# CobayaSampler/cobaya

Measured on AMD Instinct MI355X. Metric: log-posterior evals/sec (whole node), 30-dim gaussian_mixture, higher is better.
Workload: dtype f64

## Files before the change

### cobaya_amd/csrc/_exp/inc_experiment.h

```cpp
#pragma once
#include <hip/hip_runtime.h>

#define MCMC_EXP_FAMILY_STEP 0
#define MCMC_EXP_FAMILY_DRAG 1
#define MCMC_EXP_FAMILY_MIX 2
#ifndef EXP_STEP_WAVES
#define EXP_STEP_WAVES 0
#endif
#ifndef EXP_DRAG_WAVES
#define EXP_DRAG_WAVES 0
#endif
#ifndef EXP_MIX_WAVES
#define EXP_MIX_WAVES 0
#endif
#define MCMC_EXP_WAVES(family, tuned)                                                     \
    ((MCMC_EXP_FAMILY_##family == 0 && EXP_STEP_WAVES) ? EXP_STEP_WAVES                    \
     : (MCMC_EXP_FAMILY_##family == 1 && EXP_DRAG_WAVES) ? EXP_DRAG_WAVES                  \
     : (MCMC_EXP_FAMILY_##family == 2 && EXP_MIX_WAVES) ? EXP_MIX_WAVES : (tuned))
#ifdef EXP_PIPE
#define MCMC_EXP_PIPE(tuned) (EXP_PIPE)
#else
#define MCMC_EXP_PIPE(tuned) (tuned)
#endif
#ifdef EXP_ROTATE_SHIFT
#define MCMC_EXP_ROTATE_SHIFT(tuned) (EXP_ROTATE_SHIFT)
#else
#define MCMC_EXP_ROTATE_SHIFT(tuned) (tuned)
#endif
#ifdef EXP_KEEP
#define MCMC_EXP_KEEP(tuned) (EXP_KEEP != 0)
#else
#define MCMC_EXP_KEEP(tuned) (tuned)
#endif
#ifdef EXP_BOUNDS_REGS
#define MCMC_EXP_BOUNDS_LDS(tuned) (false)
#endif
#ifdef EXP_FLOAT_BOUNDS
#define MCMC_EXP_FLOAT_BOUNDS(tuned) (true)
#endif
#ifdef EXP_NO_ROTATE
#define MCMC_EXP_ROTATE(on) (false)
#else
#define MCMC_EXP_ROTATE(on) (on)
#endif

#ifdef EXP_BLOCK_TIMES
__device__ unsigned long long g_block_times[2 * 4096];
__device__ unsigned int g_wave_place[2 * 4 * 4096];
extern "C" __attribute__((visibility("default"))) int mcmc_hip_debug_block_times(unsigned long long* out)
{
    return (int)hipMemcpyFromSymbol(out, HIP_SYMBOL(g_block_times), sizeof(g_block_times));
}
extern "C" __attribute__((visibility("default"))) int mcmc_hip_debug_wave_place(unsigned int* out)
{
    return (int)hipMemcpyFromSymbol(out, HIP_SYMBOL(g_wave_place), sizeof(g_wave_place));
}
#define MCMC_EXP_BLOCK_BEGIN()                                                                \
    do {                                                                                      \
        if (threadIdx.x == 0 && blockIdx.x < 4096) g_block_times[2 * blockIdx.x] = wall_clock64(); \
        if ((threadIdx.x & 63) == 0 && blockIdx.x < 4096) {                                   \
            g_wave_place[2 * (4 * blockIdx.x + (threadIdx.x >> 6))] =                         \
                __builtin_amdgcn_s_getreg((4) | (0 << 6) | (31 << 11));                       \
            g_wave_place[2 * (4 * blockIdx.x + (threadIdx.x >> 6)) + 1] =                     \
                __builtin_amdgcn_s_getreg((20) | (0 << 6) | (31 << 11));                      \
        }                                                                                     \
    } while (0)
#define MCMC_EXP_BLOCK_END()                                                                  \
    do {                                                                                      \
        if (threadIdx.x == 0 && blockIdx.x < 4096)                                            \
            g_block_times[2 * blockIdx.x + 1] = wall_clock64();                               \
    } while (0)
#else
#define MCMC_EXP_BLOCK_BEGIN() ((void)0)
#define MCMC_EXP_BLOCK_END() ((void)0)
#endif
#ifdef EXP_FLOAT_LDS
#define MCMC_EXP_FLOAT_LDS(tuned) (EXP_FLOAT_LDS != 0)
#endif
#ifdef EXP_FLOAT_LDS_KEEP
#define MCMC_EXP_FLOAT_LDS_KEEP(tuned) (EXP_FLOAT_LDS_KEEP != 0)
#endif
#ifdef EXP_FLOAT_VEC
#define MCMC_EXP_FLOAT_VEC(tuned) (EXP_FLOAT_VEC != 0)
#endif
#ifdef EXP_DUO_DEPK
#define MCMC_DUO_DEPK(tuned) (EXP_DUO_DEPK)
#endif
#ifdef EXP_DUO_KEEPV
#define MCMC_DUO_KEEPV(tuned) (EXP_DUO_KEEPV != 0)
#endif
```

### cobaya_amd/csrc/incremental_duo.hip

```cpp
#include <string>

#include "incremental_common.h"

#ifndef MCMC_DUO_DEPK
#define MCMC_DUO_DEPK(tuned) (tuned)
#endif
#ifndef MCMC_DUO_KEEPV
#define MCMC_DUO_KEEPV(tuned) (tuned)
#endif

namespace mcmc {
namespace {

__device__ __forceinline__ double pair_swap(double v) { return quad_perm<0xB1>(v); }
__device__ __forceinline__ double duo_sum(double p_even, double p_odd)
{
    const double s = p_even + p_odd;
    return s + pair_swap(s);
}
__device__ __forceinline__ unsigned pair_max_u32(unsigned v)
{
    const unsigned o = (unsigned)__builtin_amdgcn_mov_dpp((int)v, 0xB1, 0xf, 0xf, true);
    return v > o ? v : o;
}
__device__ __forceinline__ unsigned long long pair_all_mask(unsigned long long m)
{
    m &= m >> 1;
    m &= 0x5555555555555555ull;
    return m * 3ull;
}

constexpr int kDuoRow = 33;
constexpr int kDuoStagedPairs = 4 * 8 * kDuoRow;
struct DuoVariates {
    unsigned base, off;
    __device__ __forceinline__ void init(const pair_t* sRE, int wave, int lane)
    {
        base = lds_offset(sRE + (wave * 8 * kDuoRow + (lane >> 1)));
        off = base;
    }
    __device__ __forceinline__ void put(pair_t* sRE, int wave, int lane, int h, int q, const PairRng& p)
    {
        pair_t* const mine = sRE + ((wave * 8 + 4 * h + 2 * q) * kDuoRow + (lane >> 1));
        mine[0] = pair_t{p.r[0], p.Ea[0]};
        mine[kDuoRow] = pair_t{p.r[1], p.Ea[1]};
    }
    __device__ __forceinline__ void seek(unsigned long long S) { off = base + (unsigned)(S & 7ull) * (16u * kDuoRow); }
    __device__ __forceinline__ void fetch(double& r, double& Ea) const
    {
        const pair_t re = *(lds_pairs)(unsigned long long)off;
        r = re.x;
        Ea = re.y;
    }
    __device__ __forceinline__ void next() { off += 16u * kDuoRow; }
};

__host__ __device__ constexpr int duo_chunk_mix(int dq, int km)
{
    const int avail = 80 * 1024 - 16896 - 2560 - 2048 - (duo_x_in_lds(km, dq) ? dq * 4096 : 0);
    int c = ((avail / 16) / ((1 + km) * 4 * dq)) & ~3;
    return c < 4 ? 4 : (c > 64 ? 64 : c);
}
__host__ __device__ constexpr bool duo_keep_v(int dq, int km)
{
    return 2 * dq * (km + (duo_x_in_lds(km, dq) ? 0 : 1)) + 2 * dq <= 64;
}

template <int DQ, int KM, bool UNIT_T, bool BOX0>
__global__ void __launch_bounds__(256, 2) step_duo_mix_kernel(const IncStepArgs a)
{
    extern __shared__ __attribute__((aligned(16))) double smem[];
    constexpr int dpad = 4 * DQ;
    constexpr int NE = 2 * DQ;
    constexpr int COL = (1 + KM) * dpad;
    constexpr int C = duo_chunk_mix(DQ, KM);
    constexpr int CHUNK = C * COL;
    constexpr int DEPK = MCMC_DUO_DEPK(DQ / 2);
    constexpr bool XLDS = duo_x_in_lds(KM, DQ);
    constexpr bool KEEPV = MCMC_DUO_KEEPV(duo_keep_v(DQ, KM));
    const StepArgs& s = a.s;
    const int tid = threadIdx.x, h = tid & 1, wave = tid >> 6, lane = tid & 63;
    const int W = s.W, d = a.d;
    const int w = blockIdx.x * 128 + (tid >> 1);
    const int g = __builtin_amdgcn_readfirstlane(w / s.group_size);
    const int ncols = s.n_steps;
    const double* __restrict__ gVU = a.VU + (size_t)g * ncols * COL;
    auto stage = [&](int k) {
        const int first = k * C;
        if (first >= ncols) return;
        const int cols = ncols - first < C ? ncols - first : C;
        const int bytes = cols * COL * 8;
        const char* src = (const char*)(gVU + (size_t)first * COL);
        char* dst = (char*)(smem + (k & 1) * CHUNK);
        for (int kb = wave; kb * 1024 < bytes; kb += 4) {
            if (kb * 1024 + lane * 16 < bytes)
                __builtin_amdgcn_global_load_lds(
                    (const __attribute__((address_space(1))) void*)(src + kb * 1024 + lane * 16),
                    (__attribute__((address_space(3))) void*)(dst + kb * 1024), 16, 0, 0);
        }
    };
    stage(0);
    __shared__ double2 sLH[BOX0 ? 1 : 4 * DQ];
    __shared__ double2 sNA[BOX0 ? 1 : 4 * DQ];
    __shared__ double sNM[BOX0 ? 1 : 4 * DQ];
    if (!BOX0)
        for (int i = tid; i < dpad; i += 256) {
            sLH[i] = make_double2(a.prior[i], a.prior[dpad + i]);
            sNA[i] = make_double2(a.prior[2 * dpad + i], a.prior[3 * dpad + i]);
            sNM[i] = a.prior[4 * dpad + i];
        }
    double x[XLDS ? 1 : NE], y[KM][NE];
    typedef pair_t __attribute__((address_space(3))) * lds_pairs_rw;
    __shared__ pair_t sX[XLDS ? DQ * 256 : 1];
    const unsigned xoff0 = lds_offset(sX + tid);
#pragma unroll
    for (int kk = 0; kk < DQ; ++kk) {
        double xe[2];
#pragma unroll
        for (int j = 0; j < 2; ++j) {
            const int e = 2 * kk + j, i = 4 * kk + 2 * h + j;
            const bool in = i < d;
            xe[j] = in ? s.x[(size_t)i * W + w] : (BOX0 ? 0.5 * a.box_hi : 0.0);
            if (!XLDS) x[XLDS ? 0 : e] = xe[j];
#pragma unroll
            for (int k = 0; k < KM; ++k) y[k][e] = in ? a.y[((size_t)k * d + i) * W + w] : 0.0;
        }
        if (XLDS) sX[kk * 256 + tid] = pair_t{xe[0], xe[1]};
    }
    double cn[KM], wk[KM];
#pragma unroll
    for (int k = 0; k < KM; ++k) { cn[k] = s.cblock[a.cnorm_off + k]; wk[k] = s.cblock[a.weight_off + k]; }
    double lpost = s.logpost[w], lpri = s.logprior[w], llik = s.loglike[w];
    int wt = s.weight[w], prej = s.prior_rej[w], burn = s.burn_left[w];
    const long long nacc0 = s.n_accept[w];
    int nacc = 0;
    const uint32_t gid = s.walker0 + (uint32_t)w;
    const double mt10 = s.max_tries * 10.0;
    const int lim1 = s.max_tries < 2.0e9 ? (int)floor(s.max_tries) : 0x7fffffff;
    const int lim10 = mt10 < 2.0e9 ? (int)floor(mt10) : 0x7fffffff;
    __shared__ dpair_t short_log_lds[SHORT_LOG_TABLE_SIZE];
    const short_log_tab slog = short_log_load(short_log_lds);
    __shared__ double exp64_lds[64];
    const exp_tab etab = exp_tab_load(exp64_lds);
    asm volatile("s_waitcnt vmcnt(0)" ::: "memory");
    __syncthreads();
    const unsigned long long half1 = 0xAAAAAAAAAAAAAAAAull;
    auto lse = [&](const double (&ak)[KM]) {
        double amax = ak[0];
#pragma unroll
        for (int k = 1; k < KM; ++k) amax = fmax(ak[k], amax);
        const double mine = sel(half1, ak[1], ak[0]);
        const double e_mine = dexp_tab(mine - amax, etab);
        double Ssum = fma(wk[0], quad_perm<0xA0>(e_mine), 0.0);
        Ssum = fma(wk[1], quad_perm<0xF5>(e_mine), Ssum);
        if (KM > 2) {
            const double mine2 = KM > 3 ? sel(half1, ak[3 < KM ? 3 : 0], ak[2 < KM ? 2 : 0]) : ak[2 < KM ? 2 : 0];
            const double e2 = dexp_tab(mine2 - amax, etab);
            Ssum = fma(wk[2 < KM ? 2 : 0], quad_perm<0xA0>(e2), Ssum);
            if (KM > 3) Ssum = fma(wk[3 < KM ? 3 : 0], quad_perm<0xF5>(e2), Ssum);
        }
        return dlog_tab(Ssum, slog) + amax;
    };
    double am[KM];
#pragma unroll
    for (int k = 0; k < KM; ++k) am[k] = a.amode[(size_t)k * W + w];
    if (a.anchor) {
#pragma unroll
        for (int k = 0; k < KM; ++k) {
            double pa0 = 0.0, pa1 = 0.0;
#pragma unroll
            for (int kk = 0; kk < DQ; ++kk) {
                pa0 = fma(y[k][2 * kk], y[k][2 * kk], pa0);
                pa1 = fma(y[k][2 * kk + 1], y[k][2 * kk + 1], pa1);
            }
            am[k] = -0.5 * (cn[k] + duo_sum(pa0, pa1));
        }
        llik = lse(am);
        lpost = lpri + llik;
    }
    const cdoubles gUU = (cdoubles)(unsigned long long)(a.UU + (size_t)g * ncols * KM);
    const unsigned bhi_word = (unsigned)__double2hiint(a.box_hi);
    const int hw_slot = hw_wave_slot();
    bool burning = lanes(burn > 0) != 0ull;
    unsigned long long cur_oct = ~0ull;
    __shared__ pair_t sRE[kDuoStagedPairs];
    DuoVariates sv;
    sv.init(sRE, wave, lane);

    for (int base = 0, kc = 0; base < ncols; base += C, ++kc) {
        const double* __restrict__ cur = smem + (kc & 1) * CHUNK;
        stage(kc + 1);
        const int cols = __builtin_amdgcn_readfirstlane(ncols - base < C ? ncols - base : C);
        unsigned coff = lds_offset(cur + 2 * h);
#pragma unroll 1
        for (int sl = 0; sl < cols; ++sl, coff += COL * 8) {
            const unsigned long long S = s.step0 + (unsigned long long)(base + sl);
            if ((S >> 3) != cur_oct) {
                cur_oct = S >> 3;
                rotate_priority<2>(hw_slot);
#pragma unroll 1
                for (int q = 0; q < 2; ++q) {
                    PairRng pr;
                    pr.run(s.key0, s.key1, gid, (cur_oct << 2) + (unsigned long long)(2 * h + q), slog);
                    sv.put(sRE, wave, lane, h, q, pr);
                }
                sv.seek(S);
            }
            double r, Ea;
            sv.fetch(r, Ea);
            sv.next();
            const lds_pairs col = (lds_pairs)(unsigned long long)coff;
            unsigned long long inb = ~0ull;
            double sc0 = 0.0, sc1 = 0.0;
            double dep;
            pair_t vk[KEEPV ? DQ : 1];
            unsigned xo = xoff0;
            if (XLDS) asm volatile("" : "+v"(xo));
            const lds_pairs xs = (lds_pairs)(unsigned long long)xo;
            auto xpair = [&](int kk) {
                if constexpr (XLDS) return xs[kk * 256];
                else return pair_t{x[2 * kk], x[2 * kk + 1]};
            };
            if constexpr (BOX0) {
                unsigned hmx = 0u;
#pragma unroll
                for (int kk = 0; kk < DQ; ++kk) {
                    const pair_t v = col[2 * kk];
                    const pair_t xp = xpair(kk);
                    if (KEEPV) vk[kk] = v;
                    if (kk == DEPK) dep = fma(r, v.x, xp.x);
                    const unsigned h0 = (unsigned)__double2hiint(fma(r, v.x, xp.x));
                    const unsigned h1 = (unsigned)__double2hiint(fma(r, v.y, xp.y));
                    hmx = hmx > h0 ? hmx : h0;
                    hmx = hmx > h1 ? hmx : h1;
                }
                inb = lanes(pair_max_u32(hmx) < bhi_word);
                if (inb != lanes(true)) {
                    unsigned xoff = coff;
                    asm volatile("" : "+v"(xoff));
                    const lds_pairs colx = (lds_pairs)(unsigned long long)xoff;
                    inb = ~0ull;
#pragma unroll
                    for (int kk = 0; kk < DQ; ++kk) {
                        const pair_t v = colx[2 * kk];
                        const pair_t xp = xpair(kk);
                        const double t0 = fma(r, v.x, xp.x), t1 = fma(r, v.y, xp.y);
                        inb &= lanes(t0 <= a.box_hi) & lanes(t0 >= 0.0);
                        inb &= lanes(t1 <= a.box_hi) & lanes(t1 >= 0.0);
                    }
                }
            } else {
#pragma unroll
                for (int kk = 0; kk < DQ; ++kk) {
                    const pair_t v = col[2 * kk];
                    const pair_t xp = xpair(kk);
                    if (KEEPV) vk[kk] = v;
#pragma unroll
                    for (int j = 0; j < 2; ++j) {
                        const int i = 4 * kk + 2 * h + j;
                        const double t = fma(r, j ? v.y : v.x, j ? xp.y : xp.x);
                        if (kk == DEPK && j == 0) dep = t;
                        const double2 lh = sLH[i];
                        inb &= lanes(t <= lh.y) & lanes(t >= lh.x);
                        if (a.has_norm) {
                            const double2 li = sNA[i];
                            const double qq = (t - li.x) * li.y;
                            if (j) sc1 = sc1 + fma(-0.5 * qq, qq, sNM[i]);
                            else sc0 = sc0 + fma(-0.5 * qq, qq, sNM[i]);
                        }
                    }
                }
            }
            double ak[KM];
#pragma unroll
            for (int k = 0; k < KM; ++k) {
                unsigned uoff = coff + (unsigned)((1 + k) * dpad * 8);
                asm volatile("" : "+v"(uoff) : "v"(dep));
                const lds_pairs uk = (lds_pairs)(unsigned long long)uoff;
                double pc0 = 0.0, pc1 = 0.0;
#pragma unroll
                for (int kk = 0; kk < DQ; ++kk) {
                    const pair_t u = uk[2 * kk];
                    pc0 = fma(y[k][2 * kk], u.x, pc0);
                    pc1 = fma(y[k][2 * kk + 1], u.y, pc1);
                    if (kk == DEPK) dep = pc0;
                }
                const double yu = duo_sum(pc0, pc1);
                const double uu = gUU[(size_t)(base + sl) * KM + k];
                ak[k] = fma(-0.5 * r, fma(r, uu, yu + yu), am[k]);
            }
            const unsigned long long inside_m = pair_all_mask(inb);
            const double lp = s.uniform_logp + ((!BOX0 && a.has_norm) ? duo_sum(sc0, sc1) : 0.0);
            const double ll = lse(ak);
            const double lt = lp + ll;
            const double delta = UNIT_T ? (lpost - lt) : (lpost - lt) / s.temperature;
            const unsigned long long acc_m = inside_m & (lanes(lt > lpost) | lanes(Ea > delta));
            const bool accept = __builtin_amdgcn_inverse_ballot_w64(acc_m);
            int lim = lim1;
            if (burning) {
                lim = burn > 0 ? lim10 : lim1;
                burn -= (accept & (burn > 0)) ? 1 : 0;
                burning = lanes(burn > 0) != 0ull;
            }
            const double ra = sel(acc_m, r, 0.0);
            if constexpr (XLDS) {
                unsigned xw = xoff0, poff = coff;
                asm volatile("" : "+v"(xw), "+v"(poff) : "v"(ra));
                const lds_pairs_rw px = (lds_pairs_rw)(unsigned long long)xw;
                const lds_pairs pv = (lds_pairs)(unsigned long long)poff;
#pragma unroll
                for (int kk = 0; kk < DQ; ++kk) {
                    pair_t xp = px[kk * 256];
                    pair_t v;
                    if constexpr (KEEPV) v = vk[kk];
                    else v = pv[2 * kk];
                    xp.x = fma(ra, v.x, xp.x);
                    xp.y = fma(ra, v.y, xp.y);
                    px[kk * 256] = xp;
                }
            } else if constexpr (KEEPV) {
#pragma unroll
                for (int kk = 0; kk < DQ; ++kk) {
                    x[2 * kk] = fma(ra, vk[kk].x, x[2 * kk]);
                    x[2 * kk + 1] = fma(ra, vk[kk].y, x[2 * kk + 1]);
                }
            } else {
                unsigned poff = coff;
                asm volatile("" : "+v"(poff) : "v"(ra));
                const lds_pairs pv = (lds_pairs)(unsigned long long)poff;
#pragma unroll
                for (int kk = 0; kk < DQ; ++kk) {
                    const pair_t v = pv[2 * kk];
                    x[2 * kk] = fma(ra, v.x, x[2 * kk]);
                    x[2 * kk + 1] = fma(ra, v.y, x[2 * kk + 1]);
                }
            }
#pragma unroll
            for (int k = 0; k < KM; ++k) {
                unsigned poff = coff + (unsigned)((1 + k) * dpad * 8);
                asm volatile("" : "+v"(poff) : "v"(k == 0 ? ((KEEPV || XLDS) ? ra : x[XLDS ? 0 : 2 * DEPK]) : y[k > 0 ? k - 1 : 0][2 * DEPK]));
                const lds_pairs pu = (lds_pairs)(unsigned long long)poff;
#pragma unroll
                for (int kk = 0; kk < DQ; ++kk) {
                    const pair_t u = pu[2 * kk];
                    y[k][2 * kk] = fma(ra, u.x, y[k][2 * kk]);
                    y[k][2 * kk + 1] = fma(ra, u.y, y[k][2 * kk + 1]);
                }
            }
#pragma unroll
            for (int k = 0; k < KM; ++k) am[k] = sel(acc_m, ak[k], am[k]);
            lpri = sel(acc_m, lp, lpri);
            llik = sel(acc_m, ll, llik);
            lpost = sel(acc_m, lt, lpost);
            prej = sel(acc_m, 0, prej + sel(inside_m, 0, 1));
            wt = sel(acc_m, 1, wt + 1);
            nacc += sel(acc_m, 1, 0);
            if (wt - prej > lim && h == 0) atomicCAS(s.stuck, 0, 1 + (int)gid);
        }
        asm volatile("s_waitcnt vmcnt(0)" ::: "memory");
        __syncthreads();
    }
    int we = w, he = h;
    unsigned xe_off = xoff0;
    asm volatile("" : "+v"(we), "+v"(he), "+v"(xe_off));
    const lds_pairs xend = (lds_pairs)(unsigned long long)xe_off;
#pragma unroll
    for (int e = 0; e < NE; ++e) {
        const int i = 4 * (e >> 1) + 2 * he + (e & 1);
        if (i < d) {
            double xv;
            if constexpr (XLDS) { const pair_t xp = xend[(e >> 1) * 256]; xv = (e & 1) ? xp.y : xp.x; }
            else xv = x[XLDS ? 0 : e];
            s.x[(size_t)i * W + we] = xv;
#pragma unroll
            for (int k = 0; k < KM; ++k) a.y[((size_t)k * d + i) * W + we] = y[k][e];
        }
    }
    if (h == 0) {
#pragma unroll
        for (int k = 0; k < KM; ++k) a.amode[(size_t)k * W + we] = am[k];
        s.logpost[we] = lpost; s.logprior[we] = lpri; s.loglike[we] = llik;
        s.weight[we] = wt; s.prior_rej[we] = prej; s.burn_left[we] = burn;
        s.n_accept[we] = nacc0 + nacc;
    }
    wave_add_accepts(s.accept_total, (h == 0) ? nacc : 0);
}

template <int DQ, int KM>
hipError_t launch_duo_mix(const IncStepArgs& a, hipStream_t st)
{
    constexpr int C = duo_chunk_mix(DQ, KM);
    const size_t lds = sizeof(double) * 2 * C * (1 + KM) * 4 * DQ;
    const bool unit_t = a.s.temperature == 1.0;
    typedef void (*kern_t)(const IncStepArgs);
    const bool box0 = a.box && a.box_lo == 0.0 && a.box_hi > 0.0 && a.box_hi < INFINITY;
    static const kern_t kerns[4] = {
        step_duo_mix_kernel<DQ, KM, false, false>, step_duo_mix_kernel<DQ, KM, true, false>,
        step_duo_mix_kernel<DQ, KM, false, true>, step_duo_mix_kernel<DQ, KM, true, true>};
    const std::string stem = "mcmc::step_duo_mix_kernel<" + std::to_string(DQ) + ", " + std::to_string(KM);
    static const std::string names[4] = {stem + ", false>", stem + ", true>", stem + ", false, box>",
                                         stem + ", true, box>"};
    const int v = (unit_t ? 1 : 0) + (box0 ? 2 : 0);
    if (lds > 40 * 1024) {
        hipError_t e = hipFuncSetAttribute((const void*)kerns[v],
                                           hipFuncAttributeMaxDynamicSharedMemorySize, (int)lds);
        if (e != hipSuccess) return e;
    }
    mcmc_hip_note_step_kernel(names[v].c_str());
    hipLaunchKernelGGL(kerns[v], dim3(a.s.W / 128), dim3(256), lds, st, a);
    return hipGetLastError();
}

template <int DQ>
hipError_t dispatch_duo_mix(const IncStepArgs& a, hipStream_t st)
{
    if constexpr (DQ > MCMC_DUO_DQ_HI) {
        return hipErrorInvalidValue;
    } else {
        if (a.dq == DQ) {
            if (!duo_serves(a.n_modes, DQ)) return hipErrorInvalidValue;
            if constexpr (duo_serves(4, DQ)) {
                if (a.n_modes == 4) return launch_duo_mix<DQ, 4>(a, st);
            }
            if constexpr (duo_serves(3, DQ)) {
                if (a.n_modes == 3) return launch_duo_mix<DQ, 3>(a, st);
            }
            return a.n_modes == 2 ? launch_duo_mix<DQ, 2>(a, st) : hipErrorInvalidValue;
        }
        return dispatch_duo_mix<DQ + 1>(a, st);
    }
}

#if MCMC_DUO_DQ_LO == 1
#ifndef MCMC_DUO1_SPLIT
#define MCMC_DUO1_SPLIT 1
#endif
template <bool SPLIT>
__host__ __device__ constexpr int duo1_off(int e) { return SPLIT ? 2 * e : 4 * (e >> 1) + (e & 1); }
template <bool SPLIT>
__device__ __forceinline__ int duo1_dim(int e, int h) { return duo1_off<SPLIT>(e) + (SPLIT ? h : 2 * h); }
template <bool SPLIT>
__device__ __forceinline__ double duo1_sum(double q0, double q1)
{
    if constexpr (SPLIT) {
        const double lo = q0 + pair_swap(q0), hi = q1 + pair_swap(q1);
        return lo + hi;
    } else {
        return duo_sum(q0, q1);
    }
}
__host__ __device__ constexpr int duo1_chunk(int dq)
{
    int c = ((80 * 1024 - 16896 - 2048) / (2 * 64 * dq)) & ~3;
    return c > 64 ? 64 : c;
}

template <int DQ, int NE, bool SPLIT, bool UNIT_T>
__global__ void __launch_bounds__(256, 2) step_inc_duo_kernel(const IncStepArgs a)
{
    extern __shared__ __attribute__((aligned(16))) double2 smem2[];
    constexpr int COLB = 4 * DQ, dpad = 4 * DQ;
    constexpr int C = duo1_chunk(DQ);
    constexpr int CHUNK = C * COLB;
    static_assert(SPLIT ? (NE == 2 * DQ || NE == 2 * DQ - 1) : NE == 2 * DQ, "dimensions per lane");
    const StepArgs& s = a.s;
    const int tid = threadIdx.x, h = tid & 1, wave = tid >> 6, lane = tid & 63;
    const int W = s.W, d = a.d;
    const int w = blockIdx.x * 128 + (tid >> 1);
    const int g = __builtin_amdgcn_readfirstlane(w / s.group_size);
    const int ncols = s.n_steps;
    const int set_cols = a.vu_cols > 0 ? a.vu_cols : ncols;
    const double2* __restrict__ gVU = (const double2*)a.VU + ((size_t)g * set_cols + (size_t)a.col0) * COLB;
    auto stage = [&](int k) {
        const int first = k * C;
        if (first >= ncols) return;
        const int cols = ncols - first < C ? ncols - first : C;
        const int bytes = cols * COLB * 16;
        const char* src = (const char*)(gVU + (size_t)first * COLB);
        char* dst = (char*)(smem2 + (k & 1) * CHUNK);
        for (int kb = wave; kb * 1024 < bytes; kb += 4) {
            if (kb * 1024 + lane * 16 < bytes)
                __builtin_amdgcn_global_load_lds(
                    (const __attribute__((address_space(1))) void*)(src + kb * 1024 + lane * 16),
                    (__attribute__((address_space(3))) void*)(dst + kb * 1024), 16, 0, 0);
        }
    };
    const bool refresh_y = (a.anchor & 2) != 0;
    if (!refresh_y) stage(0);
    const double blo = a.box_lo, bhi = a.box_hi;
    const unsigned bhi_word = (unsigned)__double2hiint(bhi);
    double x[NE], y[NE];
#pragma unroll
    for (int e = 0; e < NE; ++e) {
        const int i = duo1_dim<SPLIT>(e, h);
        const bool in = i < d;
        x[e] = in ? s.x[(size_t)i * W + w] : 0.5 * (blo + bhi);
        y[e] = in ? a.y[(size_t)i * W + w] : 0.0;
    }
    double lpost = s.logpost[w], lpri = s.logprior[w], llik = s.loglike[w];
    __shared__ pair_t sRE[kDuoStagedPairs];
    if (refresh_y) {
        constexpr int TW = 8, SD = (dpad + TW - 1) / TW * TW;
        static_assert(128 * SD <= 4 * CHUNK, "the chunk buffers hold the deviations of the workgroup's walkers");
        static_assert(sizeof(pair_t) * kDuoStagedPairs >= sizeof(double) * dpad * TW, "the tile fits sRE");
        double* const sdev = (double*)smem2 + (size_t)(tid >> 1) * SD;
        double* const tile = (double*)sRE;
        for (int i = h; i < SD; i += 2) sdev[i] = 0.0;
#pragma unroll
        for (int e = 0; e < NE; ++e) {
            const int i = duo1_dim<SPLIT>(e, h);
            if (i < d) sdev[i] = x[e] - a.mean[i];
            y[e] = 0.0;
        }
        for (int i0 = 0; i0 < d; i0 += TW) {
            __syncthreads();
            for (int e = tid; e < dpad * TW; e += 256) {
                const int j = e / TW, i = i0 + e % TW;
                tile[e] = (j < d && i < d) ? a.Lrow[(size_t)j * d + i] : 0.0;
            }
            __syncthreads();
            const lds_doubles pt = relaunder(tile + (SPLIT ? h : 2 * h) * TW), pd = relaunder(sdev + i0);
#pragma unroll
            for (int ii = 0; ii < TW; ++ii) {
                const double dv = pd[ii];
#pragma unroll
                for (int e = 0; e < NE; ++e) y[e] = fma(pt[duo1_off<SPLIT>(e) * TW + ii], dv, y[e]);
            }
        }
        __syncthreads();
        stage(0);
    }
    if (a.anchor) {
        double pa0 = 0.0, pa1 = 0.0;
#pragma unroll
        for (int e = 0; e < NE; ++e) {
            if (e & 1) pa1 = fma(y[e], y[e], pa1);
            else pa0 = fma(y[e], y[e], pa0);
        }
        llik = -0.5 * (s.cnorm0 + duo1_sum<SPLIT>(pa0, pa1));
        lpost = lpri + llik;
    }
    int wt = s.weight[w], prej = s.prior_rej[w], burn = s.burn_left[w];
    const long long nacc0 = s.n_accept[w];
    int nacc = 0;
    const cdoubles gUU = (cdoubles)(unsigned long long)(a.UU + (size_t)g * set_cols + (size_t)a.col0);
    const uint32_t gid = s.walker0 + (uint32_t)w;
    const double mt10 = s.max_tries * 10.0;
    const int lim1 = s.max_tries < 2.0e9 ? (int)floor(s.max_tries) : 0x7fffffff;
    const int lim10 = mt10 < 2.0e9 ? (int)floor(mt10) : 0x7fffffff;
    __shared__ dpair_t short_log_lds[SHORT_LOG_TABLE_SIZE];
    const short_log_tab slog = short_log_load(short_log_lds);
    asm volatile("s_waitcnt vmcnt(0)" ::: "memory");
    __syncthreads();
    bool burning = lanes(burn > 0) != 0ull;
    unsigned long long cur_oct = ~0ull;
    DuoVariates sv;
    sv.init(sRE, wave, lane);
    const int hw_slot = hw_wave_slot();

    for (int base = 0, k = 0; base < ncols; base += C, ++k) {
        const double2* __restrict__ cur = smem2 + (k & 1) * CHUNK;
        stage(k + 1);
        const int cols = __builtin_amdgcn_readfirstlane(ncols - base < C ? ncols - base : C);
        unsigned coff = lds_offset(cur + (SPLIT ? h : 2 * h));
#pragma unroll 1
        for (int sl = 0; sl < cols; ++sl, coff += COLB * 16) {
            const unsigned long long S = s.step0 + (unsigned long long)(base + sl);
            if ((S >> 3) != cur_oct) {
                cur_oct = S >> 3;
                rotate_priority<2>(hw_slot);
#pragma unroll 1
                for (int q = 0; q < 2; ++q) {
                    PairRng pr;
                    pr.run(s.key0, s.key1, gid, (cur_oct << 2) + (unsigned long long)(2 * h + q), slog);
                    sv.put(sRE, wave, lane, h, q, pr);
                }
                sv.seek(S);
            }
            double r, Ea;
            sv.fetch(r, Ea);
            sv.next();
            const double uu = gUU[base + sl];
            pair_t pk[NE];
            const lds_pairs col = (lds_pairs)(unsigned long long)coff;
#pragma unroll
            for (int e = 0; e < NE; ++e) pk[e] = col[duo1_off<SPLIT>(e)];
            unsigned hmx = 0u;
            double pc0 = 0.0, pc1 = 0.0;
#pragma unroll
            for (int e = 0; e < NE; ++e) {
                const double t = fma(r, pk[e].x, x[e]);
                const unsigned hw = (unsigned)__double2hiint(t);
                hmx = hmx > hw ? hmx : hw;
                if (e & 1) pc1 = fma(y[e], pk[e].y, pc1);
                else pc0 = fma(y[e], pk[e].y, pc0);
            }
            unsigned long long inside_m = lanes(pair_max_u32(hmx) < bhi_word);
            if (inside_m != lanes(true)) {
                unsigned long long inb = ~0ull;
#pragma unroll
                for (int e = 0; e < NE; ++e) {
                    const double t = fma(r, pk[e].x, x[e]);
                    inb &= lanes(t <= bhi) & lanes(t >= blo);
                }
                inside_m = pair_all_mask(inb);
            }
            const double yu = duo1_sum<SPLIT>(pc0, pc1);
            const double mhr = -0.5 * r;
            const double lp = s.uniform_logp;
            const double ll = fma(mhr, fma(r, uu, yu + yu), llik);
            const double lt = lp + ll;
            const double delta = UNIT_T ? (lpost - lt) : (lpost - lt) / s.temperature;
            const unsigned long long acc_m = inside_m & (lanes(lt > lpost) | lanes(Ea > delta));
            const bool accept = __builtin_amdgcn_inverse_ballot_w64(acc_m);
            llik = accept ? ll : llik;
            int lim = lim1;
            if (burning) {
                lim = burn > 0 ? lim10 : lim1;
                burn -= (accept & (burn > 0)) ? 1 : 0;
                burning = lanes(burn > 0) != 0ull;
            }
            const double ra = accept ? r : 0.0;
#pragma unroll
            for (int e = 0; e < NE; ++e) {
                x[e] = fma(ra, pk[e].x, x[e]);
                y[e] = fma(ra, pk[e].y, y[e]);
            }
            lpost = accept ? lt : lpost;
            {
                const bool inside = __builtin_amdgcn_inverse_ballot_w64(inside_m);
                prej = accept ? 0 : (prej + (inside ? 0 : 1));
                wt = accept ? 1 : wt + 1;
                nacc += accept ? 1 : 0;
            }
            if (wt - prej > lim && h == 0) atomicCAS(s.stuck, 0, 1 + (int)gid);
        }
        asm volatile("s_waitcnt vmcnt(0)" ::: "memory");
        __syncthreads();
    }
    int we = w, he = h;
    asm volatile("" : "+v"(we), "+v"(he));
#pragma unroll
    for (int e = 0; e < NE; ++e) {
        const int i = duo1_dim<SPLIT>(e, he);
        if (i < d) {
            s.x[(size_t)i * W + we] = x[e];
            a.y[(size_t)i * W + we] = y[e];
        }
    }
    if (h == 0) {
        s.logpost[we] = lpost; s.logprior[we] = lpri; s.loglike[we] = llik;
        s.weight[we] = wt; s.prior_rej[we] = prej; s.burn_left[we] = burn;
        s.n_accept[we] = nacc0 + nacc;
    }
    wave_add_accepts(s.accept_total, (h == 0) ? nacc : 0);
}

template <int DQ, int NE, bool SPLIT>
hipError_t launch_duo1(const IncStepArgs& a, hipStream_t st)
{
    constexpr int C = duo1_chunk(DQ);
    const size_t lds = sizeof(double2) * 2 * C * 4 * DQ;
    const bool unit_t = a.s.temperature == 1.0;
    typedef void (*kern_t)(const IncStepArgs);
    static const kern_t kerns[2] = {step_inc_duo_kernel<DQ, NE, SPLIT, false>,
                                    step_inc_duo_kernel<DQ, NE, SPLIT, true>};
    static const std::string names[2] = {"mcmc::step_inc_kernel<" + std::to_string(DQ) + ", 0, false, two lanes>",
                                         "mcmc::step_inc_kernel<" + std::to_string(DQ) + ", 0, true, two lanes>"};
    const int v = unit_t ? 1 : 0;
    if (lds > 40 * 1024) {
        hipError_t e = hipFuncSetAttribute((const void*)kerns[v],
                                           hipFuncAttributeMaxDynamicSharedMemorySize, (int)lds);
        if (e != hipSuccess) return e;
    }
    mcmc_hip_note_step_kernel(names[v].c_str());
    hipLaunchKernelGGL(kerns[v], dim3(a.s.W / 128), dim3(256), lds, st, a);
    return hipGetLastError();
}

template <int DQ>
hipError_t dispatch_duo1(const IncStepArgs& a, hipStream_t st)
{
    if constexpr (DQ > kDuo1MaxDq) {
        return hipErrorInvalidValue;
    } else {
        if (a.dq != DQ) return dispatch_duo1<DQ + 1>(a, st);
        constexpr bool SPLIT = MCMC_DUO1_SPLIT != 0;
        if constexpr (SPLIT) {
            if ((a.d + 1) / 2 == 2 * DQ - 1) return launch_duo1<DQ, 2 * DQ - 1, true>(a, st);
            return launch_duo1<DQ, 2 * DQ, true>(a, st);
        } else {
            return launch_duo1<DQ, 2 * DQ, false>(a, st);
        }
    }
}
#endif

}
}

#define MCMC_CAT2(a, b) a##b
#define MCMC_CAT(a, b) MCMC_CAT2(a, b)
extern "C" hipError_t MCMC_CAT(mcmc_hip_launch_inc_duo_, MCMC_DUO_DQ_LO)(const mcmc::IncStepArgs* a,
                                                                       hipStream_t st)
{
    if (a->dq < MCMC_DUO_DQ_LO || a->dq > MCMC_DUO_DQ_HI || a->n_drag > 0 || a->colflag || a->s.rows ||
        a->s.W % 128 != 0 || a->s.group_size % 128 != 0)
        return hipErrorInvalidValue;
    for (int q = 0; q < 4; ++q)
        if (a->periodic_mask4[q]) return hipErrorInvalidValue;
    if (a->n_modes < 2 || !a->amode || a->vu_cols > 0) return hipErrorInvalidValue;
    return mcmc::dispatch_duo_mix<MCMC_DUO_DQ_LO>(*a, st);
}

#if MCMC_DUO_DQ_LO == 1
extern "C" hipError_t mcmc_hip_launch_inc_duo1(const mcmc::IncStepArgs* a, hipStream_t st)
{
    if (a->dq < 1 || a->dq > mcmc::kDuo1MaxDq || a->n_modes != 1 || a->n_drag > 0 || a->colflag || a->s.rows ||
        a->s.W % 128 != 0 || a->s.group_size % 128 != 0 || a->has_norm || !a->box || a->box_lo != 0.0 || !a->UU)
        return hipErrorInvalidValue;
    for (int q = 0; q < 4; ++q)
        if (a->periodic_mask4[q]) return hipErrorInvalidValue;
    return mcmc::dispatch_duo1<1>(*a, st);
}
#endif
```

Baseline: 85.40 billion.

## Stage UU scalars in LDS and software-prefetch next step's column operands

Adds a second async global-to-LDS copy that stages the per-column UU scalars next to the VU chunk buffers, and shrinks the chunk size so the extra LDS fits. The inner step loop is restructured into a two-buffer ping-pong: for small per-lane dimension counts, the next column's pair data, variates and UU value are requested from LDS while the current step's accept logic runs, hiding LDS latency behind the serial Metropolis chain. It also adds optional timestamp instrumentation behind a macro. Costs are higher register pressure from the doubled operand arrays and slightly smaller chunks, meaning more barriers.

```diff
diff --git a/cobaya_amd/csrc/_exp/inc_experiment.h b/cobaya_amd/csrc/_exp/inc_experiment.h
--- a/cobaya_amd/csrc/_exp/inc_experiment.h
+++ b/cobaya_amd/csrc/_exp/inc_experiment.h
@@ -89,3 +89,34 @@
 #ifdef EXP_DUO_KEEPV
 #define MCMC_DUO_KEEPV(tuned) (EXP_DUO_KEEPV != 0)
 #endif
+#ifdef EXP_DUO1_PREFETCH
+#define MCMC_DUO1_PREFETCH(tuned) (EXP_DUO1_PREFETCH != 0)
+#endif
+#ifdef EXP_DUO1_STAMPS
+__device__ unsigned long long g_duo1_clocks[8];
+extern "C" __attribute__((visibility("default"))) int mcmc_hip_debug_duo1_clocks(unsigned long long* out, int reset)
+{
+    int rc = (int)hipMemcpyFromSymbol(out, HIP_SYMBOL(g_duo1_clocks), sizeof(g_duo1_clocks));
+    if (rc == 0 && reset) {
+        const unsigned long long zero[8] = {0, 0, 0, 0, 0, 0, 0, 0};
+        rc = (int)hipMemcpyToSymbol(HIP_SYMBOL(g_duo1_clocks), zero, sizeof(zero));
+    }
+    return rc;
+}
+#define MCMC_DUO1_STAMP_BEGIN()                                                   \
+    unsigned long long stamp_acc_[7] = {0, 0, 0, 0, 0, 0, 0};                     \
+    unsigned long long stamp_last_ = __builtin_amdgcn_s_memtime()
+#define MCMC_DUO1_STAMP(phase)                                                    \
+    do {                                                                          \
+        const unsigned long long t_ = __builtin_amdgcn_s_memtime();               \
+        stamp_acc_[phase] += t_ - stamp_last_;                                    \
+        stamp_last_ = t_;                                                         \
+    } while (0)
+#define MCMC_DUO1_STAMP_END()                                                     \
+    do {                                                                          \
+        if ((threadIdx.x & 63) == 0) {                                            \
+            for (int p_ = 0; p_ < 7; ++p_) atomicAdd(&g_duo1_clocks[p_], stamp_acc_[p_]); \
+            atomicAdd(&g_duo1_clocks[7], 1ull);                                   \
+        }                                                                         \
+    } while (0)
+#endif
diff --git a/cobaya_amd/csrc/incremental_duo.hip b/cobaya_amd/csrc/incremental_duo.hip
--- a/cobaya_amd/csrc/incremental_duo.hip
+++ b/cobaya_amd/csrc/incremental_duo.hip
@@ -1,4 +1,5 @@
 #include <string>
+#include <type_traits>
 
 #include "incremental_common.h"
 
@@ -451,9 +452,19 @@
 }
 __host__ __device__ constexpr int duo1_chunk(int dq)
 {
-    int c = ((80 * 1024 - 16896 - 2048) / (2 * 64 * dq)) & ~3;
+    int c = ((80 * 1024 - 16896 - 2048) / (2 * (64 * dq + 8))) & ~3;
     return c > 64 ? 64 : c;
 }
+
+#ifndef MCMC_DUO1_PREFETCH
+#define MCMC_DUO1_PREFETCH(tuned) (tuned)
+#endif
+#ifndef MCMC_DUO1_STAMP
+#define MCMC_DUO1_STAMP(phase) ((void)0)
+#define MCMC_DUO1_STAMP_BEGIN() ((void)0)
+#define MCMC_DUO1_STAMP_END() ((void)0)
+#endif
+__host__ __device__ constexpr bool duo1_prefetch(int ne) { return MCMC_DUO1_PREFETCH(ne <= 15); }
 
 template <int DQ, int NE, bool SPLIT, bool UNIT_T>
 __global__ void __launch_bounds__(256, 2) step_inc_duo_kernel(const IncStepArgs a)
@@ -471,6 +482,8 @@
     const int ncols = s.n_steps;
     const int set_cols = a.vu_cols > 0 ? a.vu_cols : ncols;
     const double2* __restrict__ gVU = (const double2*)a.VU + ((size_t)g * set_cols + (size_t)a.col0) * COLB;
+    const double* __restrict__ gUU = a.UU + (size_t)g * set_cols + (size_t)a.col0;
+    double* const sUU = (double*)(smem2 + 2 * CHUNK);
     auto stage = [&](int k) {
         const int first = k * C;
         if (first >= ncols) return;
@@ -484,6 +497,14 @@
                     (const __attribute__((address_space(1))) void*)(src + kb * 1024 + lane * 16),
                     (__attribute__((address_space(3))) void*)(dst + kb * 1024), 16, 0, 0);
         }
+        const char* usrc = (const char*)(gUU + first);
+        char* udst = (char*)(sUU + (k & 1) * C);
+        for (int kb = 3 - wave; kb * 256 < cols * 8; kb += 4) {
+            if (kb * 256 + lane * 4 < cols * 8)
+                __builtin_amdgcn_global_load_lds(
+                    (const __attribute__((address_space(1))) void*)(usrc + kb * 256 + lane * 4),
+                    (__attribute__((address_space(3))) void*)(udst + kb * 256), 4, 0, 0);
+        }
     };
     const bool refresh_y = (a.anchor & 2) != 0;
     if (!refresh_y) stage(0);
@@ -543,7 +564,6 @@
     int wt = s.weight[w], prej = s.prior_rej[w], burn = s.burn_left[w];
     const long long nacc0 = s.n_accept[w];
     int nacc = 0;
-    const cdoubles gUU = (cdoubles)(unsigned long long)(a.UU + (size_t)g * set_cols + (size_t)a.col0);
     const uint32_t gid = s.walker0 + (uint32_t)w;
     const double mt10 = s.max_tries * 10.0;
     const int lim1 = s.max_tries < 2.0e9 ? (int)floor(s.max_tries) : 0x7fffffff;
@@ -557,14 +577,32 @@
     DuoVariates sv;
     sv.init(sRE, wave, lane);
     const int hw_slot = hw_wave_slot();
+    MCMC_DUO1_STAMP_BEGIN();
+
+    constexpr bool PF = duo1_prefetch(NE);
+    pair_t pkA[NE], pkB[NE], reA = pair_t{0.0, 0.0}, reB = pair_t{0.0, 0.0};
+    double uuA = 0.0, uuB = 0.0;
+#pragma unroll
+    for (int e = 0; e < NE; ++e) pkA[e] = pkB[e] = pair_t{0.0, 0.0};
 
     for (int base = 0, k = 0; base < ncols; base += C, ++k) {
         const double2* __restrict__ cur = smem2 + (k & 1) * CHUNK;
         stage(k + 1);
         const int cols = __builtin_amdgcn_readfirstlane(ncols - base < C ? ncols - base : C);
         unsigned coff = lds_offset(cur + (SPLIT ? h : 2 * h));
-#pragma unroll 1
-        for (int sl = 0; sl < cols; ++sl, coff += COLB * 16) {
+        unsigned uoff = lds_offset(sUU + (k & 1) * C);
+        int sl = 0;
+        bool have = false;
+        auto request = [&](auto ahead, pair_t (&pk)[NE], pair_t& re, double& uu) __attribute__((always_inline)) {
+            constexpr int AHEAD = decltype(ahead)::value;
+            re = *(lds_pairs)(unsigned long long)(sv.off + (unsigned)(AHEAD * 16 * kDuoRow));
+            uu = *(lds_doubles)(unsigned long long)(uoff + (unsigned)(AHEAD * 8));
+            const lds_pairs col = (lds_pairs)(unsigned long long)(coff + (unsigned)(AHEAD * COLB * 16));
+#pragma unroll
+            for (int e = 0; e < NE; ++e) pk[e] = col[duo1_off<SPLIT>(e)];
+        };
+        auto step = [&](pair_t (&pk)[NE], pair_t& re, double& uuq, pair_t (&npk)[NE], pair_t& nre, double& nuu)
+                        __attribute__((always_inline)) {
             const unsigned long long S = s.step0 + (unsigned long long)(base + sl);
             if ((S >> 3) != cur_oct) {
                 cur_oct = S >> 3;
@@ -576,15 +614,14 @@
                     sv.put(sRE, wave, lane, h, q, pr);
                 }
                 sv.seek(S);
-            }
-            double r, Ea;
-            sv.fetch(r, Ea);
-            sv.next();
-            const double uu = gUU[base + sl];
-            pair_t pk[NE];
-            const lds_pairs col = (lds_pairs)(unsigned long long)coff;
-#pragma unroll
-            for (int e = 0; e < NE; ++e) pk[e] = col[duo1_off<SPLIT>(e)];
+                have = false;
+                MCMC_DUO1_STAMP(4);
+            }
+            MCMC_DUO1_STAMP(0);
+            MCMC_DUO1_STAMP(6);
+            if (!have) request(std::integral_constant<int, 0>{}, pk, re, uuq);
+            MCMC_DUO1_STAMP(5);
+            const double r = re.x, Ea = re.y, uu = uuq;
             unsigned hmx = 0u;
             double pc0 = 0.0, pc1 = 0.0;
 #pragma unroll
@@ -595,12 +632,20 @@
                 if (e & 1) pc1 = fma(y[e], pk[e].y, pc1);
                 else pc0 = fma(y[e], pk[e].y, pc0);
             }
+            MCMC_DUO1_STAMP(1);
+            if constexpr (PF) {
+                asm volatile("" : "+v"(hmx), "+v"(pc0), "+v"(pc1));
+                have = sl + 1 < cols && ((S + 1ull) & 7ull) != 0ull;
+                if (have) request(std::integral_constant<int, 1>{}, npk, nre, nuu);
+            }
             unsigned long long inside_m = lanes(pair_max_u32(hmx) < bhi_word);
             if (inside_m != lanes(true)) {
+                double rr = r;
+                asm volatile("" : "+v"(rr));
                 unsigned long long inb = ~0ull;
 #pragma unroll
                 for (int e = 0; e < NE; ++e) {
-                    const double t = fma(r, pk[e].x, x[e]);
+                    const double t = fma(rr, pk[e].x, x[e]);
                     inb &= lanes(t <= bhi) & lanes(t >= blo);
                 }
                 inside_m = pair_all_mask(inb);
@@ -621,6 +666,7 @@
                 burning = lanes(burn > 0) != 0ull;
             }
             const double ra = accept ? r : 0.0;
+            MCMC_DUO1_STAMP(2);
 #pragma unroll
             for (int e = 0; e < NE; ++e) {
                 x[e] = fma(ra, pk[e].x, x[e]);
@@ -634,6 +680,22 @@
                 nacc += accept ? 1 : 0;
             }
             if (wt - prej > lim && h == 0) atomicCAS(s.stuck, 0, 1 + (int)gid);
+            MCMC_DUO1_STAMP(3);
+            ++sl;
+            coff += COLB * 16;
+            uoff += 8;
+            sv.next();
+        };
+#pragma unroll 1
+        for (;;) {
+            if constexpr (PF) {
+                step(pkA, reA, uuA, pkB, reB, uuB);
+                if (sl == cols) break;
+                step(pkB, reB, uuB, pkA, reA, uuA);
+            } else {
+                step(pkA, reA, uuA, pkA, reA, uuA);
+            }
+            if (sl == cols) break;
         }
         asm volatile("s_waitcnt vmcnt(0)" ::: "memory");
         __syncthreads();
@@ -654,13 +716,14 @@
         s.n_accept[we] = nacc0 + nacc;
     }
     wave_add_accepts(s.accept_total, (h == 0) ? nacc : 0);
+    MCMC_DUO1_STAMP_END();
 }
 
 template <int DQ, int NE, bool SPLIT>
 hipError_t launch_duo1(const IncStepArgs& a, hipStream_t st)
 {
     constexpr int C = duo1_chunk(DQ);
-    const size_t lds = sizeof(double2) * 2 * C * 4 * DQ;
+    const size_t lds = sizeof(double2) * 2 * C * 4 * DQ + sizeof(double) * 2 * C;
     const bool unit_t = a.s.temperature == 1.0;
     typedef void (*kern_t)(const IncStepArgs);
     static const kern_t kerns[2] = {step_inc_duo_kernel<DQ, NE, SPLIT, false>,
```

Result: slower. 81.79 billion (-4.2%).
